# DoeringChristian/mitsuba3-experiments

Hardware: AMD Instinct MI355X
Metric: Mpaths/sec on bedroom@1280×720 spp=256, 1/2/4/8 GPUs; HBM GB/s vs peak (higher is better)
Workload: dtype f32; 1 GPU; path-mis.py NEE+MIS (BASELINE configs[1]) on bedroom-proxy 1280x720, global spp=256 split over 1 rank(s) by sample range, max_depth=8, rr_depth=2; global_spp=256, spp_per_rank=256, parallelism=sample-range shards x1

## Files before the change

mitsuba3-experiments_amd/csrc/context.cpp:

```cpp
#include <stdlib.h>
#include <string.h>

#include <algorithm>

#include "runtime.h"

namespace mtxh {

int dalloc(DevBuf &b, size_t bytes) {
  if (b.bytes >= bytes && b.p) return MTX_OK;
  if (b.p) hipFree(b.p);
  b.p = nullptr;
  b.bytes = 0;
  if (bytes == 0) return MTX_OK;
  hipError_t e = hipMalloc(&b.p, bytes);
  if (e != hipSuccess) {
    mtx_set_error("hipMalloc(%zu) failed: %s", bytes, hipGetErrorString(e));
    b.p = nullptr;
    return MTX_E_OOM;
  }
  b.bytes = bytes;
  return MTX_OK;
}

// ... 18 lines not shown
    if (p && !on_device(c, p)) {
      mtx_set_error("%s: argument %d is not device memory of device %d", fn, k, c->device);
      return MTX_E_ARG;
    }
    ++k;
  }
  return MTX_OK;
}

int stage(mtx_ctx *c, DevBuf &slot, size_t bytes, const void *src) {
  if (int rc = dalloc(slot, bytes)) return rc;
  if (src) HIP_TRY(hipMemcpyAsync(slot.p, src, bytes, hipMemcpyHostToDevice, c->stream));
  return MTX_OK;
}
int unstage(mtx_ctx *c, std::initializer_list<Unstage> outs) {
  for (const Unstage &o : outs) HIP_TRY(hipMemcpyAsync(o.dst, o.slot.p, o.bytes, hipMemcpyDeviceToHost, c->stream));
  HIP_TRY(hipStreamSynchronize(c->stream));
  return MTX_OK;
}

}

using namespace mtxh;

static bool read_knobs(Knobs &k) {
  if (const char *e = getenv("MTX_LDS_STACK")) k.lds_stack = std::max(1, std::min(MTX_BVH_MAX_DEPTH + 1, atoi(e)));
  if (const char *e = getenv("MTX_LDS_TOP")) k.lds_top = (uint32_t)std::max(0, std::min(256, atoi(e)));
  if (const char *e = getenv("MTX_OCC_LDS_TOP")) k.occ_lds_top = (uint32_t)std::max(0, std::min(192, atoi(e)));
  if (const char *e = getenv("MTX_OCC_LDS_STACK"))
    k.occ_lds_stack = std::max(1, std::min(MTX_BVH_MAX_DEPTH + 1, atoi(e)));
  if (const char *e = getenv("MTX_STREAMS_MAX_LOG2")) k.streams_max_log2 = (uint32_t)std::max(16, std::min(31, atoi(e)));
  if (const char *e = getenv("MTX_STREAMS")) k.streams = (uint32_t)std::max(1, std::min(2, atoi(e)));
  if (const char *e = getenv("MTX_TRACE_BATCH")) k.trace_batch = (uint32_t)std::max(1, std::min(1 << 16, atoi(e)));
  if (const char *e = getenv("MTX_UREFILL")) k.urefill = (uint32_t)std::max(1, std::min(64, atoi(e)));
  if (const char *e = getenv("MTX_CAM_UREFILL")) k.cam_urefill = (uint32_t)std::max(1, std::min(64, atoi(e)));
  if (const char *e = getenv("MTX_OCC_UREFILL")) k.occ_urefill = (uint32_t)std::max(1, std::min(64, atoi(e)));
  if (const char *e = getenv("MTX_TRACE_RING")) {
    char *end = nullptr;
    const long v = strtol(e, &end, 10);
    if (end == e || *end || !mtxd::ring_size_ok(v)) {
      mtx_set_error("MTX_TRACE_RING=%s: the ring holds 0 (none), 16 or 32 rays", e);
      return false;
    }
    k.trace_ring = (uint32_t)v;
  }
  if (const char *e = getenv("MTX_XCD_CLAIM")) k.xcd_claim = atoi(e) != 0;
  if (const char *e = getenv("MTX_RS_FUSED")) k.rs_fused = atoi(e) ? 1u : 0u;
  if (const char *e = getenv("MTX_MEGA_PATHS")) k.mega_paths = (uint32_t)strtoul(e, nullptr, 0);
  if (const char *e = getenv("MTX_CACHE_FUSED")) k.cache_fused = atoi(e) ? 1u : 0u;
  if (const char *e = getenv("MTX_ENCODE_LM")) k.encode_lm = atoi(e) ? 1u : 0u;
  if (const char *e = getenv("MTX_CACHE_SORT")) k.cache_sort = (uint32_t)std::max(0, std::min(2, atoi(e)));
  return true;
}

extern "C" {

int mtx_diag_shade_stamps(unsigned long long *out) { return mtxd::shade_stamps(out); }

int mtx_diag_trace_lds(uint32_t ring, uint32_t lds_stack, uint32_t lds_top, uint32_t *out) {
  if (!out || !mtxd::ring_size_ok(ring) || !lds_stack) return MTX_E_ARG;
  mtxd::DevScene s{};
  s.lds_entries = lds_stack;
  s.lds_top = lds_top;
  mtxd::split_trace_lds(s, ring);
  out[0] = (uint32_t)mtxd::ring_stack_bytes(s);
  out[1] = s.ring_lds_entries;
  return MTX_OK;
}

int mtx_ctx_create(int hip_device, mtx_ctx **out) {
  if (!out) {
    mtx_set_error("mtx_ctx_create: out is NULL");
    return MTX_E_ARG;
  }
  *out = nullptr;
  int n = 0;
  HIP_TRY(hipGetDeviceCount(&n));
  if (hip_device < 0 || hip_device >= n) {
    mtx_set_error("mtx_ctx_create: device %d out of range (%d devices)", hip_device, n);
    return MTX_E_ARG;
  }
  HIP_TRY(hipSetDevice(hip_device));
  hipDeviceProp_t prop;
  HIP_TRY(hipGetDeviceProperties(&prop, hip_device));
  if (strncmp(prop.gcnArchName, "gfx950", 6) != 0) {
    mtx_set_error("mtx_ctx_create: device %d is %s, libmtx is built for gfx950", hip_device, prop.gcnArchName);
    return MTX_E_UNSUPPORTED;
  }
  mtx_ctx *c = new mtx_ctx();
  c->device = hip_device;
  c->n_cu = prop.multiProcessorCount;
  hipError_t e = hipStreamCreateWithFlags(&c->stream, hipStreamNonBlocking);
  if (e != hipSuccess) {
    delete c;
    mtx_set_error("hipStreamCreate failed: %s", hipGetErrorString(e));
    return MTX_E_HIP;
  }
  c->wave[0].stream = c->stream;
  c->trace_grid = c->closest_grid = c->n_cu * 8;
  c->shade_grid = c->n_cu * mtxd::shade_blocks_per_cu();
  {
    int v = 0;
    c->max_lds = 160 * 1024;
    if (hipDeviceGetAttribute(&v, hipDeviceAttributeMaxSharedMemoryPerBlock, hip_device) == hipSuccess &&
        (size_t)v > c->max_lds)
      c->max_lds = (size_t)v;
  }
  if (!read_knobs(c->knobs)) {
    mtx_ctx_destroy(c);
    return MTX_E_ARG;
  }
  *out = c;
  return MTX_OK;
}

void mtx_ctx_destroy(mtx_ctx *c) {
  if (!c) return;
  hipSetDevice(c->device);
  for (Wave &w : c->wave)
    if (w.stream) hipStreamSynchronize(w.stream);
  Wave &w1 = c->wave[1];
  if (w1.start) hipEventDestroy(w1.start);
  if (w1.done) hipEventDestroy(w1.done);
  if (w1.stream) hipStreamDestroy(w1.stream);
  for (hipEvent_t ev : c->events) hipEventDestroy(ev);
  if (c->q_pinned) hipHostFree(c->q_pinned);
  for (hipEvent_t ev : c->prim_ev)
    if (ev) hipEventDestroy(ev);
  if (c->stream) hipStreamDestroy(c->stream);
  delete c;
}

double mtx_last_device_ms(mtx_ctx *c) { return c ? c->last_device_ms : 0.0; }

// ... 2 lines not shown
```

mitsuba3-experiments_amd/csrc/render.cpp:

```cpp
#include <string.h>

#include <algorithm>
#include <initializer_list>
#include <vector>

#include "runtime.h"
#include "mtx_core/film.h"
#include "prims.h"

namespace mtxh {

constexpr uint32_t kDefaultChunk = 1u << 28;
constexpr size_t kPathStateBytes = 328;
constexpr size_t kCacheQueryBytes = 3 * kQueryBytes + kFeatBytes + kOutBytes;
uint32_t default_chunk(mtx_ctx *c, const mtx_render_args *a, uint32_t ways, bool cache) {
  size_t free_b = 0, total_b = 0;
  if (hipMemGetInfo(&free_b, &total_b) != hipSuccess) return 1u << 22;
  const size_t per_path =
      kPathStateBytes + (cache ? kCacheQueryBytes : 0) +
      (a->integrator == MTX_INT_PSSMLT_SIMPLE ? 32ull * std::max<uint32_t>(a->max_depth, 1) + 48
       : a->integrator == MTX_INT_PSSMLT_PATH ? 48ull * std::max<uint32_t>(a->max_depth, 1) + 48
                                              : 0);
  const size_t held =
      ways > 1 ? std::min<size_t>(c->wave[0].capacity, c->wave[1].capacity) : c->wave[0].capacity;
// ... 191 lines not shown
      if (hipMemcpyAsync(&nq, b.cq_count, 4, hipMemcpyDeviceToHost, st) == hipSuccess &&
          hipStreamSynchronize(st) == hipSuccess)
        tm.cache_queries += nq;
    }
  }
  return MTX_OK;
}

void launch_bounce(mtx_ctx *c, const mtxd::WaveBuffers &b, const mtxd::ChunkParams &p, Timer &tm,
                   uint64_t *n_trace, uint64_t *n_shadow, const mtxd::DevScene &s, hipStream_t st, uint32_t bounce) {
  const bool nerad = p.integrator == MTX_INT_NERAD_RHS, nerad_render = p.integrator == MTX_INT_NERAD;
  hipEvent_t e;
  const int div = (nerad && bounce >= 2) ? 8 : 1;
  if (!(nerad && bounce == 0)) {
    e = tm.begin(0, st);
    if (bounce == 0 && p.cam0)
      mtxd::launch_trace_camera(s, b, p, std::max(1, c->closest_grid / div), st);
    else
      mtxd::launch_trace_closest(s, b, bounce, p.stats, std::max(1, c->closest_grid / div), st);
    tm.end(0, e, st);
    ++*n_trace;
  }
  e = tm.begin(2, st);
  mtxd::launch_shade(s, b, p, bounce, std::max(1, c->shade_grid / div), st);
  tm.end(2, e, st);
  if (p.integrator != MTX_INT_PSSMLT_SIMPLE && p.integrator != MTX_INT_SIMPLE && !nerad_render &&
      !(nerad && bounce > 0)) {
    e = tm.begin(1, st);
    mtxd::launch_trace_shadow(s, b, bounce, p.stats, c->trace_grid, st);
    tm.end(1, e, st);
    ++*n_shadow;
  }
}

uint32_t bounce_iters(const mtxd::ChunkParams &p) {
  return std::max<uint32_t>(p.max_depth, 1) + (p.nrc_cache ? 1u : 0u);
}

void finish_bounces(const mtxd::WaveBuffers &b, const mtxd::ChunkParams &p, hipStream_t st) {
  if (p.integrator != MTX_INT_NERAD_RHS && p.integrator != MTX_INT_NERAD)
    mtxd::launch_flush_tail(b, bounce_iters(p), b.capacity, p.integrator, st);
}

void run_bounces(mtx_ctx *c, const Wave &w, const mtxd::WaveBuffers &b, const mtxd::ChunkParams &p, Timer &tm,
                 uint64_t *n_trace, uint64_t *n_shadow) {
  const mtxd::DevScene s = wave_scene(c, w);
  hipStream_t st = w.stream;
// ... 665 lines not shown
```

mitsuba3-experiments_amd/csrc/runtime.h:

```cpp
#pragma once
#include <hip/hip_runtime.h>
#include <stdint.h>

#include <initializer_list>
#include <utility>
#include <vector>

#include "mtx.h"
#include "mtx_core/field.h"
#include "mtx_core/nerad.h"
#include "refit.h"
#include "wavefront.h"

void mtx_set_error(const char *fmt, ...);

#define HIP_TRY(expr)                                                                             \
  do {                                                                                            \
    hipError_t e_ = (expr);                                                                       \
    if (e_ != hipSuccess) {                                                                       \
      mtx_set_error("%s failed: %s (%s:%d)", #expr, hipGetErrorString(e_), __FILE__, __LINE__); \
      return MTX_E_HIP;                                                                           \
    }                                                                                             \
  } while (0)

// ... 46 lines not shown
struct Wave {
  hipStream_t stream = nullptr;
  hipEvent_t start = nullptr, done = nullptr;
  DevBuf plane[kNumPlanes];
  DevBuf counters, xheads;
  DevBuf stack_ovf;
  DevBuf cq_p, cq_d, cq_t, cq_count, f_feat, f_out;
  DevBuf cq_perm, cq_cursor;
  uint32_t capacity = 0;
};

struct Knobs {
  uint32_t streams = MTX_STREAMS;
  uint32_t streams_max_log2 = 27;
  uint32_t lds_stack = mtxd::kLdsStack;
  uint32_t lds_top = MTX_LDS_TOP;
  uint32_t occ_lds_top = MTX_OCC_LDS_TOP;
  uint32_t occ_lds_stack = mtxd::kOccLdsStack;
  uint32_t trace_batch = 128;
  uint32_t urefill = 24;
  uint32_t cam_urefill = 64;
  uint32_t occ_urefill = 12;
  uint32_t trace_ring = MTX_TRACE_RING;
  uint32_t xcd_claim = 1;
  uint32_t mega_paths = 0xffffffffu;
  uint32_t rs_fused = 1;
  uint32_t cache_sort = MTX_CACHE_SORT;
  uint32_t encode_lm = MTX_ENCODE_LM;
  uint32_t cache_fused = 1;
};

struct SceneState {
  DevBuf shade_rec;
  DevBuf nodes, tri, occ_nodes, occ_tri, tri_vidx, tri_shape, vpos, vnormal, vuv, shapes, materials, emitters, textures,
      texels, tables;
  mtxd::DevScene dev{};
  uint32_t n_shapes = 0;
  uint32_t n_materials = 0;
  uint32_t n_nodes = 0, n_occ = 0, n_verts = 0, n_tables = 0;
  bool live = false;
};

struct RefitState {
  DevBuf occ_perm, lvl4_list, lvl8_list;
  std::vector<uint32_t> lvl4_first, lvl8_first;
  DevBuf state, tbox, nbox, vpos, vnormal;
// ... 160 lines not shown
```

mitsuba3-experiments_amd/csrc/scene.cpp:

```cpp
#include <string.h>

#include <algorithm>
#include <vector>

#include "runtime.h"
#include "mtx_core/interaction.h"
#include "scene_check.h"

using namespace mtxh;

static int upload_levels(const std::vector<uint32_t> &level, uint32_t depth, std::vector<uint32_t> &first,
                         DevBuf &list, hipStream_t st) {
  first.assign((size_t)depth + 1, 0u);
  bool contiguous = true;
  uint32_t prev = 0;
  for (uint32_t l : level) {
    if (l >= depth) {
      contiguous = false;
      continue;
    }
    ++first[l + 1];
    contiguous = contiguous && l >= prev;
    prev = l;
  }
  for (uint32_t l = 0; l < depth; ++l) first[l + 1] += first[l];
  if (contiguous) {
    dfree(list);
    return MTX_OK;
  }
// ... 89 lines not shown
    t.pmf = (float *)c->refit.em_pmf.p;
    t.cdf = (float *)c->refit.em_cdf.p;
    t.bsum = (double *)c->refit.em_bsum.p;
    t.bstat = (uint32_t *)c->refit.em_bstat.p;
  }
  {
    std::vector<float> rec(32 * (size_t)d->n_tris, 0.f);
    for (uint32_t t = 0; t < d->n_tris; ++t) {
      float *r = &rec[32 * (size_t)t];
      const mtx_shape &sh = d->shapes[d->tri_shape[t]];
      const uint32_t use_n = (!(sh.flags & 1u) && d->vnormal) ? 1u : 0u;
      const uint32_t use_uv = ((sh.flags & 2u) && d->vuv) ? 2u : 0u;
      for (int k = 0; k < 3; ++k) {
        const uint32_t vi = d->tri_vidx[3 * (size_t)t + k];
        for (int a = 0; a < 3; ++a) r[4 * k + a] = d->vpos[3 * (size_t)vi + a];
        if (use_n)
          for (int a = 0; a < 3; ++a) r[12 + 4 * k + a] = d->vnormal[3 * (size_t)vi + a];
        if (use_uv) {
          r[24 + 2 * k] = d->vuv[2 * (size_t)vi];
          r[24 + 2 * k + 1] = d->vuv[2 * (size_t)vi + 1];
        }
      }
      const mtx_material &m = d->materials[sh.material];
      const uint32_t cls = 1u + ((m.type & 7u) << 2 | (m.tex >= 0 ? 2u : 0u) | ((m.flags & MTX_MF_MASK) ? 1u : 0u));
      const uint32_t mat = sh.material, fl = use_n | use_uv | (cls << 8);
      const int32_t em = sh.emitter;
      memcpy(&r[3], &mat, 4);
      memcpy(&r[7], &em, 4);
      memcpy(&r[11], &fl, 4);
    }
    if ((rc = upload(c->scene.shade_rec, rec.data(), rec.size(), st))) return rc;
    HIP_TRY(hipStreamSynchronize(st));
  }
  HIP_TRY(hipStreamSynchronize(st));
  mtxd::DevScene &s = c->scene.dev;
  s.nodes = (const int4 *)c->scene.nodes.p;
  s.tri = (const float *)c->scene.tri.p;
  s.occ_nodes = (const int4 *)c->scene.occ_nodes.p;
  s.occ_tri = (const float *)c->scene.occ_tri.p;
  s.tri_vidx = (const uint32_t *)c->scene.tri_vidx.p;
  s.tri_shape = (const uint32_t *)c->scene.tri_shape.p;
  s.vpos = (const float *)c->scene.vpos.p;
  s.vnormal = (const float *)c->scene.vnormal.p;
  s.vuv = (const float *)c->scene.vuv.p;
  s.shapes = (const mtx_shape *)c->scene.shapes.p;
  s.shade_rec = (const float4 *)c->scene.shade_rec.p;
  s.materials = (const mtx_material *)c->scene.materials.p;
// ... 133 lines not shown
  if (e == hipSuccess) e = hipStreamSynchronize(st);
  if (e == hipSuccess) e = hipGetLastError();
  if (e != hipSuccess || (flags & mtxd::RF_BAD_QUANT)) {
    c->scene_dropped();
    if (e != hipSuccess) {
      mtx_set_error("mtx_scene_update_vertices: %s; the scene was dropped, upload it again", hipGetErrorString(e));
      return MTX_E_HIP;
    }
    mtx_set_error("mtx_scene_update_vertices: child box quantisation failed; the scene was dropped, upload it again");
    return MTX_E_ARG;
  }
  mtx::V3 lo, hi;
  lo.x = mtxd::refit_key_decode(h[mtxd::RF_LO]);
  lo.y = mtxd::refit_key_decode(h[mtxd::RF_LO + 1]);
  lo.z = mtxd::refit_key_decode(h[mtxd::RF_LO + 2]);
  hi.x = mtxd::refit_key_decode(h[mtxd::RF_HI]);
  hi.y = mtxd::refit_key_decode(h[mtxd::RF_HI + 1]);
  hi.z = mtxd::refit_key_decode(h[mtxd::RF_HI + 2]);
  mtx::env_bsphere_box(lo, hi, c->scene.dev.env_center, &c->scene.dev.env_radius);
  c->geometry_moved();
  return MTX_OK;
}

int mtx_scene_read(mtx_ctx *c, int which, void *out, uint64_t n_bytes) {
  if (!c || !out) {
    mtx_set_error("mtx_scene_read: null argument");
    return MTX_E_ARG;
  }
  if (!c->scene.live) {
    mtx_set_error("no scene uploaded");
    return MTX_E_NOSCENE;
  }
  const uint64_t nt = c->scene.dev.n_tris, nv = c->scene.n_verts;
  const void *src = nullptr;
  uint64_t need = 0;
  switch (which) {
    case 0: src = c->scene.nodes.p; need = 4ull * MTX_BVH_NODE_WORDS * c->scene.n_nodes; break;
    case 1: src = c->scene.occ_nodes.p; need = 4ull * MTX_OCC_NODE_WORDS * c->scene.n_occ; break;
    case 2: src = c->scene.tri.p; need = 36 * nt; break;
    case 3: src = c->scene.occ_tri.p; need = 36 * nt; break;
    case 4: src = c->scene.shade_rec.p; need = 128 * nt; break;
    case 5: src = c->scene.vpos.p; need = 12 * nv; break;
    case 6: src = c->scene.vnormal.p; need = c->scene.vnormal.p ? 12 * nv : 0; break;
    case 7: need = 16; break;
    case 8: src = c->scene.tables.p; need = 4ull * c->scene.n_tables; break;
    case 9: src = c->scene.emitters.p; need = sizeof(mtx_emitter) * (uint64_t)c->scene.dev.n_emitters; break;
// ... 22 lines not shown
```

mitsuba3-experiments_amd/csrc/shade.hip:

```cpp
#include <hip/hip_runtime.h>

#include <algorithm>

#include "device_common.h"
#include "shade_dev.h"

#ifndef MTX_SHADE_MIN_BLOCKS
#define MTX_SHADE_MIN_BLOCKS 3
#endif
constexpr int kShadeMinBlocks = MTX_SHADE_MIN_BLOCKS;

namespace mtxd {

__global__ void k_raygen_camera(DevScene s, WaveBuffers b, ChunkParams p) {
  const uint32_t i = blockIdx.x * blockDim.x + threadIdx.x;
  if (i == 0) b.counters[0] = p.n_paths;
  if (i >= p.n_paths) return;
  const CamPath cp = camera_path(s.camera, s.has_env != 0, p, i);
  init_path(b, p, i, cp.ray, cp.rng, cp.pos, s.has_env != 0);
}

__global__ void k_raygen_rays(DevScene s, WaveBuffers b, ChunkParams p, const float *rays, const uint32_t *lanes,
                              uint32_t rng_skip) {
  const uint32_t i = blockIdx.x * blockDim.x + threadIdx.x;
  if (i == 0) b.counters[0] = p.n_paths;
  if (i >= p.n_paths) return;
  Pcg32 rng = sampler_lane(p.seed, lanes[i]);
  for (uint32_t k = 0; k < rng_skip; ++k) rng.next_u32();
  const float *r = rays + 6 * (size_t)i;
  Ray ray{V3{r[0], r[1], r[2]}, V3{r[3], r[4], r[5]}, kLargest};
  init_path(b, p, i, ray, rng, make_float2(0.f, 0.f), s.has_env != 0);
}

#if MTX_DIAG_STAMPS
__device__ unsigned long long g_shade_stamps[kStampSegs + 2];
#endif

template <int INT, bool CAM>
__device__ __forceinline__ void shade_loop(const DevScene &s, const WaveBuffers &b, const ChunkParams &p,
                                           uint32_t bounce_) {
  const uint32_t bounce = CAM ? 0u : bounce_;
  const SceneView sv = make_view(s);
  const uint32_t count = b.counters[4 * bounce + 0];
  const uint32_t *in_q = b.queue[bounce & 1];
  uint32_t *out_q = b.queue[(bounce + 1) & 1];
  uint32_t *out_cnt = &b.counters[4 * (bounce + 1) + 0];
  const uint32_t rp = (bounce + b.ray_par) & 1u;
  constexpr bool kNerad = INT == MTX_INT_NERAD_RHS || INT == MTX_INT_NERAD;
  const uint32_t stride = gridDim.x * kShadeBlock;
  uint32_t parity = 0;
  uint32_t path = 0;
  float4 h = make_float4(0.f, 0.f, 0.f, 0.f);
  const bool ident = bounce == 0 && p.ident0;
  if (blockIdx.x * kShadeBlock + threadIdx.x < count) {
    const uint32_t i0 = blockIdx.x * kShadeBlock + threadIdx.x;
    path = ident ? i0 : ld_stream<kNtQueue>(in_q + i0);
    h = ld_stream<kNtShade>(b.hit + i0);
  }

  Stamps stp{};
  MTX_STAMP_BEGIN(stp);
  for (uint32_t base = blockIdx.x * kShadeBlock; base < count; base += stride, parity ^= 1u) {
    const uint32_t i = base + threadIdx.x;
    const uint32_t inext = i + stride;
    uint32_t path_n = 0;
    if (inext < count) path_n = ident ? inext : ld_stream<kNtQueue>(in_q + inext);
    float4 hn = make_float4(0.f, 0.f, 0.f, 0.f);
    if (inext < count) hn = b.hit[inext];
    const uint32_t pn = __float_as_uint(hn.y);
    const float4 *wp = (inext < count && pn != 0xffffffffu) ? s.shade_rec + 8 * (size_t)pn : nullptr;
    ShadeIO io;
    io.reset();
    MTX_STAMP_STEP(stp);
    io.st = stp;
    bool cont = false;
    const bool valid = i < count;
    if (valid) {
      if constexpr (INT == MTX_INT_PSSMLT_SIMPLE)
        cont = shade_pssmlt(s, sv, b, p, bounce, path, i, h, io);
      else if constexpr (INT == MTX_INT_SIMPLE)
        cont = shade_simple<CAM>(s, sv, b, p, bounce, path, i, h, io);
      else if constexpr (INT == MTX_INT_PSSMLT_PATH)
        cont = shade_pssmlt_path(s, sv, b, p, bounce, path, i, h, io);
      else if constexpr (INT == MTX_INT_NERAD_RHS)
        cont = shade_nerad<false>(s, sv, b, bounce, path, i, h, io);
      else if constexpr (INT == MTX_INT_NERAD)
        cont = shade_nerad<true>(s, sv, b, bounce, path, i, h, io);
      else
        cont = shade_path<INT, CAM>(s, sv, b, p, bounce, path, i, h, io, wp);
    }
    (void)wp;
    const uint32_t path_c = path;
    path = path_n;
    h = hn;
    asm volatile("" ::"v"(io.warm));
    stp = io.st;

    uint32_t slot, sslot;
    block_append2<kShadeBlock>(cont, io.emit, io.emit && io.em_hi, out_cnt, parity, slot, sslot);
    MTX_STAMP(stp, 6);
    if (cont) {
      st_stream<kNtQueue>(out_q + slot, path_c);
      st_stream<kNtShadeSt>(b.ray_o[rp ^ 1u] + slot, io.nro);
      st_stream<kNtShadeSt>(b.ray_d[rp ^ 1u] + slot, io.nrd);
      if constexpr (!kNerad) st_stream<kNtShadeSt>(b.thr[rp ^ 1u] + slot, io.nthr);
      if constexpr (INT == MTX_INT_PATH_MIS || INT == MTX_INT_PATH || INT == MTX_INT_NRC || INT == MTX_INT_PSSMLT_PATH)
        st_stream<kNtShadeSt>(b.prev[rp ^ 1u] + slot, io.nprev);
      if constexpr (!kNerad) {
        st_stream<kNtShadeSt>(b.L[rp ^ 1u] + slot, io.nL);
        st_stream<kNtShadeSt>(b.misc[rp ^ 1u] + slot, io.nmisc);
      }
    } else if (!kNerad && valid) {
      st_stream<kNtShadeSt>(b.L[kFinal] + path_c, io.nL);
      if (!p.drop_end_misc) st_stream<kNtShadeSt>(b.misc[kFinal] + path_c, io.nmisc);
    }
    if (io.emit) {
      const uint32_t li = (kNerad || !cont) ? kFinal * b.capacity + path_c : (rp ^ 1u) * b.capacity + slot;
      io.rec.d.w = __uint_as_float(li);
// ... 7 lines not shown
    if constexpr (INT == MTX_INT_NRC || INT == MTX_INT_NERAD_RHS || INT == MTX_INT_NERAD) {
      if (INT != MTX_INT_NRC || p.nrc_cache) {
        const uint32_t q = block_reserve<kShadeBlock>(io.query ? 1u : 0u, b.cq_count);
        if (io.query) {
          b.cq_p[q] = io.qp;
          b.cq_d[q] = io.qd;
          b.cq_t[q] = io.qt;
        }
      }
    }
    MTX_STAMP(stp, 8);
  }
#if MTX_DIAG_STAMPS
  if ((threadIdx.x & 63u) == 0) {
    for (int k = 0; k < kStampSegs; ++k) atomicAdd(&g_shade_stamps[k], stp.acc[k]);
    atomicAdd(&g_shade_stamps[kStampSegs], stp.steps);
    atomicAdd(&g_shade_stamps[kStampSegs + 1], 1ull);
  }
#endif
}

template <int INT>
__global__ __launch_bounds__(kShadeBlock, kShadeMinBlocks) void k_shade(DevScene s, WaveBuffers b, ChunkParams p, uint32_t bounce) {
  shade_loop<INT, false>(s, b, p, bounce);
}
template <int INT>
__global__ __launch_bounds__(kShadeBlock, kShadeMinBlocks) void k_shade_cam(DevScene s, WaveBuffers b, ChunkParams p) {
  static_assert(INT == MTX_INT_PATH || INT == MTX_INT_PATH_MIS || INT == MTX_INT_NRC || INT == MTX_INT_SIMPLE,
                "k_shade_cam: the integrators whose bounce-0 shade derives the camera sample");
  shade_loop<INT, true>(s, b, p, 0u);
}

__global__ void k_flush_tail(WaveBuffers b, uint32_t bounce, uint32_t integrator) {
  const uint32_t n = b.counters[4 * bounce];
  const uint32_t *q = b.queue[bounce & 1];
  const uint32_t rp = (bounce + b.ray_par) & 1u;
  for (uint32_t k = blockIdx.x * blockDim.x + threadIdx.x; k < n; k += gridDim.x * blockDim.x) {
    const uint32_t path = q[k];
    float4 L = b.L[rp][k];
    const uint4 m = b.misc[rp][k];
    if (integrator == MTX_INT_PATH_MIS || integrator == MTX_INT_RESTIR_GI) L.w = end_w(m.w >> 16);
    b.L[kFinal][path] = L;
    b.misc[kFinal][path] = m;
  }
}

// ... 83 lines not shown
    cur.y = po.y;
    b.mlt_L[i] = f4(Lp, 0.f);
    for (uint32_t d = 0; d < dirty; ++d)
      b.vpath[(size_t)d * b.capacity + i] = b.vprop[(size_t)d * b.capacity + i];
    if (p.integrator == MTX_INT_PSSMLT_PATH)
      for (uint32_t d = 0; d < dirty; ++d)
        b.vpath_es[(size_t)d * b.capacity + i] = b.vprop_es[(size_t)d * b.capacity + i];
    dirty = 0;
  }
  cur.w = (float)dirty;
  b.mlt_cur[i] = cur;
  b.misc[kFinal][i] = st_rng(rng, 0u);
}

void launch_raygen_camera(const DevScene &s, const WaveBuffers &b, const ChunkParams &p, hipStream_t st) {
  hipLaunchKernelGGL(k_raygen_camera, dim3(blocks_for(p.n_paths, 256)), dim3(256), 0, st, s, b, p);
}
void launch_raygen_rays(const DevScene &s, const WaveBuffers &b, const ChunkParams &p, const float *rays,
                        const uint32_t *lanes, uint32_t rng_skip, hipStream_t st) {
  hipLaunchKernelGGL(k_raygen_rays, dim3(blocks_for(p.n_paths, 256)), dim3(256), 0, st, s, b, p, rays, lanes,
                     rng_skip);
}
void launch_shade(const DevScene &s, const WaveBuffers &b, const ChunkParams &p, uint32_t bounce, int grid,
                  hipStream_t st) {
  if (bounce == 0 && p.cam0) {
    switch (p.integrator) {
      case MTX_INT_PATH:
        hipLaunchKernelGGL(k_shade_cam<MTX_INT_PATH>, dim3(grid), dim3(kShadeBlock), 0, st, s, b, p);
        break;
      case MTX_INT_NRC:
        hipLaunchKernelGGL(k_shade_cam<MTX_INT_NRC>, dim3(grid), dim3(kShadeBlock), 0, st, s, b, p);
        break;
      case MTX_INT_SIMPLE:
        hipLaunchKernelGGL(k_shade_cam<MTX_INT_SIMPLE>, dim3(grid), dim3(kShadeBlock), 0, st, s, b, p);
        break;
      default:
        hipLaunchKernelGGL(k_shade_cam<MTX_INT_PATH_MIS>, dim3(grid), dim3(kShadeBlock), 0, st, s, b, p);
    }
    return;
  }
  switch (p.integrator) {
    case MTX_INT_PATH:
      hipLaunchKernelGGL(k_shade<MTX_INT_PATH>, dim3(grid), dim3(kShadeBlock), 0, st, s, b, p, bounce);
      break;
    case MTX_INT_NRC:
      hipLaunchKernelGGL(k_shade<MTX_INT_NRC>, dim3(grid), dim3(kShadeBlock), 0, st, s, b, p, bounce);
      break;
    case MTX_INT_PSSMLT_SIMPLE:
      hipLaunchKernelGGL(k_shade<MTX_INT_PSSMLT_SIMPLE>, dim3(grid), dim3(kShadeBlock), 0, st, s, b, p, bounce);
      break;
    case MTX_INT_SIMPLE:
      hipLaunchKernelGGL(k_shade<MTX_INT_SIMPLE>, dim3(grid), dim3(kShadeBlock), 0, st, s, b, p, bounce);
      break;
    case MTX_INT_PSSMLT_PATH:
      hipLaunchKernelGGL(k_shade<MTX_INT_PSSMLT_PATH>, dim3(grid), dim3(kShadeBlock), 0, st, s, b, p, bounce);
      break;
    case MTX_INT_NERAD_RHS:
      hipLaunchKernelGGL(k_shade<MTX_INT_NERAD_RHS>, dim3(grid), dim3(kShadeBlock), 0, st, s, b, p, bounce);
      break;
    case MTX_INT_NERAD:
      hipLaunchKernelGGL(k_shade<MTX_INT_NERAD>, dim3(grid), dim3(kShadeBlock), 0, st, s, b, p, bounce);
      break;
    default:
      hipLaunchKernelGGL(k_shade<MTX_INT_PATH_MIS>, dim3(grid), dim3(kShadeBlock), 0, st, s, b, p, bounce);
  }
}
int shade_stamps(unsigned long long *out) {
#if MTX_DIAG_STAMPS
  if (hipDeviceSynchronize() != hipSuccess) return -1;
  if (hipMemcpyFromSymbol(out, HIP_SYMBOL(g_shade_stamps), sizeof(unsigned long long) * (kStampSegs + 2)) !=
      hipSuccess)
    return -1;
  unsigned long long z[kStampSegs + 2] = {};
  if (hipMemcpyToSymbol(HIP_SYMBOL(g_shade_stamps), z, sizeof(z)) != hipSuccess) return -1;
  return kStampSegs;
#else
  (void)out;
  return -1;
#endif
}
int shade_blocks_per_cu() {
  int nb = 0;
  if (hipOccupancyMaxActiveBlocksPerMultiprocessor(&nb, k_shade<MTX_INT_PATH_MIS>, kShadeBlock, 0) != hipSuccess ||
      nb <= 0)
    nb = 2;
  return nb;
}
void launch_cache_apply(const WaveBuffers &b, const float *out, uint32_t capacity, hipStream_t st,
                        const uint32_t *perm) {
  const unsigned blocks = (unsigned)std::min<uint64_t>((capacity + 255) / 256, 16384);
  hipLaunchKernelGGL(k_cache_apply, dim3(std::max(1u, blocks)), dim3(256), 0, st, b, out, perm);
}
void launch_flush_tail(const WaveBuffers &b, uint32_t bounce, uint32_t capacity, uint32_t integrator,
                       hipStream_t st) {
  const unsigned blocks = (unsigned)std::min<uint64_t>((capacity + 255) / 256, 1024);
  hipLaunchKernelGGL(k_flush_tail, dim3(std::max(1u, blocks)), dim3(256), 0, st, b, bounce, integrator);
}
void launch_mlt_init(const WaveBuffers &b, const ChunkParams &p, hipStream_t st) {
  hipLaunchKernelGGL(k_mlt_init, dim3(blocks_for(p.n_paths, 256)), dim3(256), 0, st, b, p, p.max_depth);
}
void launch_mlt_begin(const DevScene &s, const WaveBuffers &b, const ChunkParams &p, hipStream_t st) {
  hipLaunchKernelGGL(k_mlt_begin, dim3(blocks_for(p.n_paths, 256)), dim3(256), 0, st, s, b, p);
}
void launch_mlt_end(const WaveBuffers &b, const ChunkParams &p, hipStream_t st) {
  hipLaunchKernelGGL(k_mlt_end, dim3(blocks_for(p.n_paths, 256)), dim3(256), 0, st, b, p, p.max_depth);
}

// ... 10 lines not shown
```

mitsuba3-experiments_amd/csrc/wavefront.h:

```cpp
#pragma once
#include <hip/hip_runtime.h>
#include <stdint.h>

#include "mtx.h"
#include "mtx_core/nerad.h"

namespace mtxd {

enum : uint32_t {
  PF_VALID_RAY = 1u,
  PF_PREV_DELTA = 2u,
  PF_PRIMARY_VALID = 4u,
  PF_CACHE_QUERY = 8u,
};

#ifndef MTX_TRACE_BLOCK
#define MTX_TRACE_BLOCK 256
#endif
constexpr int kTraceBlock = MTX_TRACE_BLOCK;
constexpr int kShadeBlock = 256;
constexpr uint32_t kLdsStack = 16;
constexpr uint32_t kOccLdsStack = 8;
#ifndef MTX_LDS_TOP
#define MTX_LDS_TOP 64
#endif
#ifndef MTX_OCC_LDS_TOP
#define MTX_OCC_LDS_TOP 48
#endif
#ifndef MTX_TRACE_RING
#define MTX_TRACE_RING 32
#endif
constexpr bool ring_size_ok(long R) { return R == 0 || R == 16 || R == 32; }
static_assert(ring_size_ok(MTX_TRACE_RING), "MTX_TRACE_RING: 0, 16 or 32");
constexpr uint32_t kTraceLds = 20 * 1024;
constexpr uint32_t kRingWords = 14;
constexpr uint32_t ring_bytes(uint32_t R) { return R * 4u * kRingWords * (kTraceBlock / 64u); }
#ifndef MTX_CACHE_SORT
#define MTX_CACHE_SORT 2
#endif
#ifndef MTX_ENCODE_LM
#define MTX_ENCODE_LM 1
#endif
#ifndef MTX_CAM0
#define MTX_CAM0 1
#endif
#ifndef MTX_STREAMS
#define MTX_STREAMS 2
#endif

constexpr uint32_t kXcds = 8;
constexpr uint32_t kXHeadStride = 32;
constexpr uint32_t kXSlotWords = kXcds * kXHeadStride;

struct DevScene {
  const int4 *nodes;
  const float *tri;
  const int4 *occ_nodes;
  const float *occ_tri;
  const uint32_t *tri_vidx;
// ... 116 lines not shown
struct ChunkParams {
  uint32_t integrator, max_depth, rr_depth, seed;
  uint32_t spp, spp_total, sample_offset;
  uint32_t width, height;
  uint32_t px0, n_px;
  uint32_t band_y0;
  uint32_t band_px;
  uint32_t rfilter;
  uint32_t film_slots;
  uint32_t slot_mask;
  uint32_t n_paths;
  float nrc_c;
  uint32_t stats;
  uint32_t large_step;
  uint32_t restir;
  uint32_t nrc_cache;
  uint32_t drop_end_misc;
  uint32_t ident0;
  uint32_t cam0;
};

int trace_blocks_per_cu(const DevScene &s);
int closest_blocks_per_cu(const DevScene &s);
int shade_blocks_per_cu();
int mega_blocks_per_cu(const DevScene &s);
void launch_path_mega(const DevScene &s, const WaveBuffers &b, const ChunkParams &p, int grid, hipStream_t st);
void launch_rs_stage_a(const DevScene &s, const WaveBuffers &b, const ChunkParams &p, const RestirBuffers &r,
                       int grid, hipStream_t st);
int shade_stamps(unsigned long long *out);
void launch_raygen_camera(const DevScene &s, const WaveBuffers &b, const ChunkParams &p, hipStream_t st);
void launch_raygen_rays(const DevScene &s, const WaveBuffers &b, const ChunkParams &p, const float *rays,
                        const uint32_t *lanes, uint32_t rng_skip, hipStream_t st);
void launch_trace_closest(const DevScene &s, const WaveBuffers &b, uint32_t bounce, uint32_t stats, int grid,
                          hipStream_t st);
void launch_trace_camera(const DevScene &s, const WaveBuffers &b, const ChunkParams &p, int grid, hipStream_t st);
void launch_trace_shadow(const DevScene &s, const WaveBuffers &b, uint32_t bounce, uint32_t stats, int grid,
                         hipStream_t st);
void launch_shade(const DevScene &s, const WaveBuffers &b, const ChunkParams &p, uint32_t bounce, int grid,
                  hipStream_t st);
void launch_film_src(const WaveBuffers &b, const ChunkParams &p, float4 *contrib, hipStream_t st);
void launch_film_gather(const float4 *contrib, float4 *film, uint32_t width, uint32_t y0, uint32_t y1,
                        uint32_t nslots, uint32_t slot_mask, uint32_t rfilter, hipStream_t st);
void launch_mlt_init(const WaveBuffers &b, const ChunkParams &p, hipStream_t st);
void launch_mlt_begin(const DevScene &s, const WaveBuffers &b, const ChunkParams &p, hipStream_t st);
void launch_mlt_end(const WaveBuffers &b, const ChunkParams &p, hipStream_t st);
void launch_mlt_film(const WaveBuffers &b, const ChunkParams &p, float4 *contrib, hipStream_t st);
void launch_flush_tail(const WaveBuffers &b, uint32_t bounce, uint32_t capacity, uint32_t integrator,
                       hipStream_t st);
void launch_collect(const WaveBuffers &b, const ChunkParams &p, float *L_out, uint8_t *valid_out, hipStream_t st);
void launch_cache_apply(const WaveBuffers &b, const float *out, uint32_t capacity, hipStream_t st,
                        const uint32_t *perm = nullptr);
void launch_restir_begin(const DevScene &s, const WaveBuffers &b, const ChunkParams &p, const RestirBuffers &r,
                         hipStream_t st);
void launch_restir_collect(const WaveBuffers &b, const ChunkParams &p, const RestirBuffers &r, hipStream_t st);
void launch_restir_temporal(const RestirBuffers &r, const ChunkParams &p, hipStream_t st);
void launch_restir_spatial_rays(const RestirBuffers &r, const ChunkParams &p, hipStream_t st);
void launch_restir_spatial_merge(const RestirBuffers &r, const ChunkParams &p, hipStream_t st);
void launch_restir_bias_finish(const RestirBuffers &r, const ChunkParams &p, hipStream_t st);
void launch_restir_final(const DevScene &s, const WaveBuffers &b, const ChunkParams &p, const RestirBuffers &r,
                         hipStream_t st);
void launch_trace_test(const DevScene &s, const RestirBuffers &r, uint32_t occ_base, int grid, hipStream_t st);
void launch_trace_raw(const DevScene &s, const float4 *rays, uint32_t n, int any_hit, uint32_t *hits,
// ... 10 lines not shown
```

Before: 1546 Mpaths/s.

## Bin shade work into per-material-class LDS ring queues to cut divergence

Adds an in-block compaction scheme to the shade kernel for path and path-mis integrators. Each block ballots incoming hits by material class (diffuse, roughplastic, other), stages them in per-class LDS rings, and shades a full block of a single class whenever one fills, flushing mixed leftovers at the end. The aim is to cut wavefront divergence across material BSDF code paths. In exchange it adds LDS use that can lower occupancy, extra block barriers per batch, and it drops the next-item prefetch of the mixed loop. It is on by default and can be disabled with an env knob.

After: 1760 Mpaths/s, median of 6. 13.9% higher.

```diff
diff --git a/include/mtx_core/shade_class.h b/include/mtx_core/shade_class.h
--- /dev/null
+++ b/include/mtx_core/shade_class.h
@@ -0,0 +1,21 @@
+#pragma once
+#include "../mtx.h"
+#include "common.h"
+
+namespace mtx {
+
+constexpr uint32_t kShadeClasses = 3;
+
+MTX_HD uint32_t shade_class_of_type(uint32_t type) {
+  return type == MTX_MAT_DIFFUSE ? 0u : type == MTX_MAT_ROUGHPLASTIC ? 1u : 2u;
+}
+
+MTX_HD uint32_t shade_rec_class_bits(uint32_t type, bool textured, bool masked) {
+  return 1u + ((type & 7u) << 2 | (textured ? 2u : 0u) | (masked ? 1u : 0u));
+}
+MTX_HD uint32_t shade_class_of_rec(uint32_t flag_word) {
+  const uint32_t c = (flag_word >> 8) & 0x1fu;
+  return c ? shade_class_of_type((c - 1u) >> 2) : 0u;
+}
+
+}
diff --git a/mitsuba3-experiments_amd/csrc/context.cpp b/mitsuba3-experiments_amd/csrc/context.cpp
--- a/mitsuba3-experiments_amd/csrc/context.cpp
+++ b/mitsuba3-experiments_amd/csrc/context.cpp
@@ -64,6 +64,15 @@
 }
 
 using namespace mtxh;
+
+static bool shade_classes_knob(const char *e, uint32_t *out) {
+  if (!e || !(e[0] == '0' || e[0] == '1') || e[1]) {
+    mtx_set_error("MTX_SHADE_CLASSES=%s: 0 (the mixed shade loop) or 1 (class queues)", e ? e : "(null)");
+    return false;
+  }
+  *out = (uint32_t)(e[0] - '0');
+  return true;
+}
 
 static bool read_knobs(Knobs &k) {
   if (const char *e = getenv("MTX_LDS_STACK")) k.lds_stack = std::max(1, std::min(MTX_BVH_MAX_DEPTH + 1, atoi(e)));
@@ -86,6 +95,9 @@
     }
     k.trace_ring = (uint32_t)v;
   }
+  if (const char *e = getenv("MTX_SHADE_CLASSES")) {
+    if (!shade_classes_knob(e, &k.shade_classes)) return false;
+  }
   if (const char *e = getenv("MTX_XCD_CLAIM")) k.xcd_claim = atoi(e) != 0;
   if (const char *e = getenv("MTX_RS_FUSED")) k.rs_fused = atoi(e) ? 1u : 0u;
   if (const char *e = getenv("MTX_MEGA_PATHS")) k.mega_paths = (uint32_t)strtoul(e, nullptr, 0);
@@ -98,6 +110,8 @@
 extern "C" {
 
 int mtx_diag_shade_stamps(unsigned long long *out) { return mtxd::shade_stamps(out); }
+
+int mtx_diag_shade_class_mix(unsigned long long *out) { return mtxd::shade_class_mix(out); }
 
 int mtx_diag_trace_lds(uint32_t ring, uint32_t lds_stack, uint32_t lds_top, uint32_t *out) {
   if (!out || !mtxd::ring_size_ok(ring) || !lds_stack) return MTX_E_ARG;
@@ -110,6 +124,22 @@
   return MTX_OK;
 }
 
+uint32_t mtx_diag_shade_class_of_type(uint32_t type) { return mtx::shade_class_of_type(type); }
+int mtx_diag_shade_classes_knob(const char *value, uint32_t *out) {
+  if (!out || !shade_classes_knob(value, &out[0])) return MTX_E_ARG;
+  out[1] = mtxd::shade_class_lds_bytes();
+  out[2] = mtxd::kClassRing;
+  out[3] = mtx::kShadeClasses;
+  return MTX_OK;
+}
+
+int mtx_diag_shade_grid(const mtx_ctx *c, uint32_t *out) {
+  if (!c || !out) return MTX_E_ARG;
+  out[0] = (uint32_t)c->shade_grid;
+  out[1] = (uint32_t)c->n_cu;
+  return MTX_OK;
+}
+
 int mtx_ctx_create(int hip_device, mtx_ctx **out) {
   if (!out) {
     mtx_set_error("mtx_ctx_create: out is NULL");
@@ -140,7 +170,6 @@
   }
   c->wave[0].stream = c->stream;
   c->trace_grid = c->closest_grid = c->n_cu * 8;
-  c->shade_grid = c->n_cu * mtxd::shade_blocks_per_cu();
   {
     int v = 0;
     c->max_lds = 160 * 1024;
@@ -152,6 +181,7 @@
     mtx_ctx_destroy(c);
     return MTX_E_ARG;
   }
+  c->shade_grid = c->n_cu * mtxd::shade_blocks_per_cu(c->knobs.shade_classes != 0);
   *out = c;
   return MTX_OK;
 }
diff --git a/mitsuba3-experiments_amd/csrc/render.cpp b/mitsuba3-experiments_amd/csrc/render.cpp
--- a/mitsuba3-experiments_amd/csrc/render.cpp
+++ b/mitsuba3-experiments_amd/csrc/render.cpp
@@ -237,7 +237,7 @@
     ++*n_trace;
   }
   e = tm.begin(2, st);
-  mtxd::launch_shade(s, b, p, bounce, std::max(1, c->shade_grid / div), st);
+  mtxd::launch_shade(s, b, p, bounce, std::max(1, c->shade_grid / div), st, c->knobs.shade_classes != 0);
   tm.end(2, e, st);
   if (p.integrator != MTX_INT_PSSMLT_SIMPLE && p.integrator != MTX_INT_SIMPLE && !nerad_render &&
       !(nerad && bounce > 0)) {
diff --git a/mitsuba3-experiments_amd/csrc/runtime.h b/mitsuba3-experiments_amd/csrc/runtime.h
--- a/mitsuba3-experiments_amd/csrc/runtime.h
+++ b/mitsuba3-experiments_amd/csrc/runtime.h
@@ -92,6 +92,7 @@
   uint32_t cam_urefill = 64;
   uint32_t occ_urefill = 12;
   uint32_t trace_ring = MTX_TRACE_RING;
+  uint32_t shade_classes = MTX_SHADE_CLASSES;
   uint32_t xcd_claim = 1;
   uint32_t mega_paths = 0xffffffffu;
   uint32_t rs_fused = 1;
diff --git a/mitsuba3-experiments_amd/csrc/scene.cpp b/mitsuba3-experiments_amd/csrc/scene.cpp
--- a/mitsuba3-experiments_amd/csrc/scene.cpp
+++ b/mitsuba3-experiments_amd/csrc/scene.cpp
@@ -5,6 +5,7 @@
 
 #include "runtime.h"
 #include "mtx_core/interaction.h"
+#include "mtx_core/shade_class.h"
 #include "scene_check.h"
 
 using namespace mtxh;
@@ -140,7 +141,7 @@
         }
       }
       const mtx_material &m = d->materials[sh.material];
-      const uint32_t cls = 1u + ((m.type & 7u) << 2 | (m.tex >= 0 ? 2u : 0u) | ((m.flags & MTX_MF_MASK) ? 1u : 0u));
+      const uint32_t cls = mtx::shade_rec_class_bits(m.type, m.tex >= 0, (m.flags & MTX_MF_MASK) != 0);
       const uint32_t mat = sh.material, fl = use_n | use_uv | (cls << 8);
       const int32_t em = sh.emitter;
       memcpy(&r[3], &mat, 4);
@@ -320,6 +321,24 @@
   return MTX_OK;
 }
 
+int mtx_diag_shade_classes(const mtx_scene_desc *d, uint8_t *out) {
+  if (!d || !out || !d->tri_shape || !d->shapes || !d->materials) {
+    mtx_set_error("mtx_diag_shade_classes: null argument");
+    return MTX_E_ARG;
+  }
+  for (uint32_t t = 0; t < d->n_tris; ++t) {
+    const uint32_t sh = d->tri_shape[t];
+    if (sh >= d->n_shapes || d->shapes[sh].material >= d->n_materials) {
+      mtx_set_error("mtx_diag_shade_classes: triangle %u: shape or material out of range", t);
+      return MTX_E_ARG;
+    }
+    const mtx_material &m = d->materials[d->shapes[sh].material];
+    const uint32_t fl = mtx::shade_rec_class_bits(m.type, m.tex >= 0, (m.flags & MTX_MF_MASK) != 0) << 8;
+    out[t] = (uint8_t)mtx::shade_class_of_rec(fl);
+  }
+  return MTX_OK;
+}
+
 int mtx_scene_read(mtx_ctx *c, int which, void *out, uint64_t n_bytes) {
   if (!c || !out) {
     mtx_set_error("mtx_scene_read: null argument");
diff --git a/mitsuba3-experiments_amd/csrc/shade.hip b/mitsuba3-experiments_amd/csrc/shade.hip
--- a/mitsuba3-experiments_amd/csrc/shade.hip
+++ b/mitsuba3-experiments_amd/csrc/shade.hip
@@ -36,9 +36,34 @@
 __device__ unsigned long long g_shade_stamps[kStampSegs + 2];
 #endif
 
-template <int INT, bool CAM>
+#ifndef MTX_DIAG_CLASSES
+#define MTX_DIAG_CLASSES 0
+#endif
+#if MTX_DIAG_CLASSES
+constexpr uint32_t kMixBounces = 16, kMixWords = 2 * mtx::kShadeClasses;
+__device__ unsigned long long g_class_mix[kMixBounces][kMixWords];
+__device__ __forceinline__ void class_mix_count(const DevScene &s, uint32_t bounce, bool valid, const float4 h) {
+  const uint32_t prim = __float_as_uint(h.y);
+  uint32_t cw = 0;
+  if (valid && prim != 0xffffffffu) cw = __float_as_uint(s.shade_rec[8 * (size_t)prim + 2].w);
+  const uint32_t cls = mtx::shade_class_of_rec(cw);
+  uint32_t held = 0, n[mtx::kShadeClasses];
+  for (uint32_t k = 0; k < mtx::kShadeClasses; ++k) {
+    n[k] = (uint32_t)__popcll(__ballot(valid && cls == k));
+    held += n[k] ? 1u : 0u;
+  }
+  if ((threadIdx.x & 63u) == 0 && held && bounce < kMixBounces) {
+    atomicAdd(&g_class_mix[bounce][held - 1], 1ull);
+    for (uint32_t k = 0; k < mtx::kShadeClasses; ++k)
+      atomicAdd(&g_class_mix[bounce][mtx::kShadeClasses + k], (unsigned long long)n[k]);
+  }
+}
+#endif
+
+template <int INT, bool CAM, bool CLS = false>
 __device__ __forceinline__ void shade_loop(const DevScene &s, const WaveBuffers &b, const ChunkParams &p,
                                            uint32_t bounce_) {
+  static_assert(!CLS || (shade_has_classes(INT) && !CAM), "class queues: k_shade of path-mis and path");
   const uint32_t bounce = CAM ? 0u : bounce_;
   const SceneView sv = make_view(s);
   const uint32_t count = b.counters[4 * bounce + 0];
@@ -57,43 +82,163 @@
     path = ident ? i0 : ld_stream<kNtQueue>(in_q + i0);
     h = ld_stream<kNtShade>(b.hit + i0);
   }
+  constexpr uint32_t kC = mtx::kShadeClasses, kW = kShadeBlock / 64, kMask = kClassRing - 1;
+  static_assert((kClassRing & kMask) == 0 && kClassRing >= 2 * kShadeBlock, "a ring holds two block steps");
+  static_assert(kClassEntryBytes == sizeof(float4) + sizeof(uint2), "ring entry: hit record | position, path");
+  extern __shared__ float4 class_lds[];
+  float4 *ring_h = class_lds;
+  uint2 *ring_ip = reinterpret_cast<uint2 *>(class_lds + kC * kClassRing);
+  __shared__ uint32_t class_wcnt[CLS ? kW : 1][kC];
+  uint32_t head[kC] = {}, fill[kC] = {};
+  uint32_t nbase = blockIdx.x * kShadeBlock, cw = 0;
+  bool cw_due = CLS && nbase < count;
+  auto load_class_word = [&]() {
+    const uint32_t pn = __float_as_uint(h.y);
+    cw = 0;
+    if (nbase + threadIdx.x < count && pn != 0xffffffffu) cw = __float_as_uint(s.shade_rec[8 * (size_t)pn + 2].w);
+    cw_due = false;
+  };
 
   Stamps stp{};
   MTX_STAMP_BEGIN(stp);
-  for (uint32_t base = blockIdx.x * kShadeBlock; base < count; base += stride, parity ^= 1u) {
-    const uint32_t i = base + threadIdx.x;
-    const uint32_t inext = i + stride;
-    uint32_t path_n = 0;
-    if (inext < count) path_n = ident ? inext : ld_stream<kNtQueue>(in_q + inext);
-    float4 hn = make_float4(0.f, 0.f, 0.f, 0.f);
-    if (inext < count) hn = b.hit[inext];
-    const uint32_t pn = __float_as_uint(hn.y);
-    const float4 *wp = (inext < count && pn != 0xffffffffu) ? s.shade_rec + 8 * (size_t)pn : nullptr;
+  for (uint32_t base = blockIdx.x * kShadeBlock; CLS || base < count; base += CLS ? 0u : stride, parity ^= 1u) {
+    uint32_t i = base + threadIdx.x, path_s = path, path_n = 0;
+    float4 h_s = h, hn = make_float4(0.f, 0.f, 0.f, 0.f);
+    bool valid = i < count;
+    const float4 *wp = nullptr;
+    if constexpr (!CLS) {
+      const uint32_t inext = i + stride;
+      if (inext < count) path_n = ident ? inext : ld_stream<kNtQueue>(in_q + inext);
+      if (inext < count) hn = b.hit[inext];
+      const uint32_t pn = __float_as_uint(hn.y);
+      wp = (inext < count && pn != 0xffffffffu) ? s.shade_rec + 8 * (size_t)pn : nullptr;
+    } else {
+      const uint32_t wave = threadIdx.x >> 6;
+      uint32_t c, most, held;
+      for (;;) {
+        c = 0;
+        most = held = fill[0];
+#pragma unroll
+        for (uint32_t k = 1; k < kC; ++k) {
+          if (fill[k] > most) {
+            most = fill[k];
+            c = k;
+          }
+          held += fill[k];
+        }
+        if (most >= (uint32_t)kShadeBlock || nbase >= count) break;
+        if (cw_due) load_class_word();
+        const uint32_t i_n = nbase + threadIdx.x;
+        const bool in = i_n < count;
+        const uint32_t cls = mtx::shade_class_of_rec(cw);
+        uint64_t m[kC];
+#pragma unroll
+        for (uint32_t k = 0; k < kC; ++k) m[k] = __ballot(in && cls == k);
+        if ((threadIdx.x & 63u) == 0) {
+#pragma unroll
+          for (uint32_t k = 0; k < kC; ++k) class_wcnt[wave][k] = (uint32_t)__popcll(m[k]);
+        }
+        __syncthreads();
+        uint32_t slot = 0;
+#pragma unroll
+        for (uint32_t k = 0; k < kC; ++k) {
+          uint32_t before = 0, total = 0;
+#pragma unroll
+          for (uint32_t w = 0; w < kW; ++w) {
+            const uint32_t n = __builtin_amdgcn_readfirstlane(class_wcnt[w][k]);
+            if (w < wave) before += n;
+            total += n;
+          }
+          const uint32_t rank = before + __builtin_amdgcn_mbcnt_hi((uint32_t)(m[k] >> 32),
+                                                                   __builtin_amdgcn_mbcnt_lo((uint32_t)m[k], 0u));
+          if (cls == k) slot = k * kClassRing + ((head[k] + fill[k] + rank) & kMask);
+          fill[k] += total;
+        }
+        if (in) {
+          ring_h[slot] = h;
+          ring_ip[slot] = make_uint2(i_n, path);
+        }
+        nbase += stride;
+        if (nbase + threadIdx.x < count) {
+          path = ident ? nbase + threadIdx.x : ld_stream<kNtQueue>(in_q + nbase + threadIdx.x);
+          h = b.hit[nbase + threadIdx.x];
+        }
+        cw_due = nbase < count;
+        __syncthreads();
+      }
+      if (held == 0) break;
+      valid = false;
+      if (most >= (uint32_t)kShadeBlock) {
+        uint32_t hc = 0;
+#pragma unroll
+        for (uint32_t k = 0; k < kC; ++k)
+          if (c == k) {
+            hc = head[k];
+            head[k] = (head[k] + kShadeBlock) & kMask;
+            fill[k] -= kShadeBlock;
+          }
+        const uint32_t slot = c * kClassRing + ((hc + threadIdx.x) & kMask);
+        const uint2 ip = ring_ip[slot];
+        h_s = ring_h[slot];
+        i = ip.x;
+        path_s = ip.y;
+        valid = true;
+      } else {
+        uint32_t t = threadIdx.x, room = kShadeBlock;
+#pragma unroll
+        for (uint32_t k = 0; k < kC; ++k) {
+          const uint32_t take = fill[k] < room ? fill[k] : room;
+          if (!valid && t < take) {
+            const uint32_t slot = k * kClassRing + ((head[k] + t) & kMask);
+            const uint2 ip = ring_ip[slot];
+            h_s = ring_h[slot];
+            i = ip.x;
+            path_s = ip.y;
+            valid = true;
+          }
+          t -= take;
+          head[k] = (head[k] + take) & kMask;
+          fill[k] -= take;
+          room -= take;
+        }
+      }
+#pragma unroll
+      for (uint32_t k = 0; k < kC; ++k) {
+        head[k] = __builtin_amdgcn_readfirstlane(head[k]);
+        fill[k] = __builtin_amdgcn_readfirstlane(fill[k]);
+      }
+    }
     ShadeIO io;
     io.reset();
     MTX_STAMP_STEP(stp);
     io.st = stp;
     bool cont = false;
-    const bool valid = i < count;
+#if MTX_DIAG_CLASSES
+    if constexpr (!CAM && !CLS && shade_has_classes(INT)) class_mix_count(s, bounce, valid, h_s);
+#endif
     if (valid) {
       if constexpr (INT == MTX_INT_PSSMLT_SIMPLE)
-        cont = shade_pssmlt(s, sv, b, p, bounce, path, i, h, io);
+        cont = shade_pssmlt(s, sv, b, p, bounce, path_s, i, h_s, io);
       else if constexpr (INT == MTX_INT_SIMPLE)
-        cont = shade_simple<CAM>(s, sv, b, p, bounce, path, i, h, io);
+        cont = shade_simple<CAM>(s, sv, b, p, bounce, path_s, i, h_s, io);
       else if constexpr (INT == MTX_INT_PSSMLT_PATH)
-        cont = shade_pssmlt_path(s, sv, b, p, bounce, path, i, h, io);
+        cont = shade_pssmlt_path(s, sv, b, p, bounce, path_s, i, h_s, io);
       else if constexpr (INT == MTX_INT_NERAD_RHS)
-        cont = shade_nerad<false>(s, sv, b, bounce, path, i, h, io);
+        cont = shade_nerad<false>(s, sv, b, bounce, path_s, i, h_s, io);
       else if constexpr (INT == MTX_INT_NERAD)
-        cont = shade_nerad<true>(s, sv, b, bounce, path, i, h, io);
+        cont = shade_nerad<true>(s, sv, b, bounce, path_s, i, h_s, io);
       else
-        cont = shade_path<INT, CAM>(s, sv, b, p, bounce, path, i, h, io, wp);
+        cont = shade_path<INT, CAM>(s, sv, b, p, bounce, path_s, i, h_s, io, wp);
     }
     (void)wp;
-    const uint32_t path_c = path;
-    path = path_n;
-    h = hn;
-    asm volatile("" ::"v"(io.warm));
+    const uint32_t path_c = path_s;
+    if constexpr (!CLS) {
+      path = path_n;
+      h = hn;
+      asm volatile("" ::"v"(io.warm));
+    } else {
+      if (cw_due) load_class_word();
+    }
     stp = io.st;
 
     uint32_t slot, sslot;
@@ -147,6 +292,11 @@
 
 template <int INT>
 __global__ __launch_bounds__(kShadeBlock, kShadeMinBlocks) void k_shade(DevScene s, WaveBuffers b, ChunkParams p, uint32_t bounce) {
+  shade_loop<INT, false, shade_has_classes(INT)>(s, b, p, bounce);
+}
+template <int INT>
+__global__ __launch_bounds__(kShadeBlock, kShadeMinBlocks) void k_shade_mixed(DevScene s, WaveBuffers b, ChunkParams p, uint32_t bounce) {
+  static_assert(shade_has_classes(INT), "k_shade_mixed: the integrators whose k_shade runs class queues");
   shade_loop<INT, false>(s, b, p, bounce);
 }
 template <int INT>
@@ -276,7 +426,8 @@
                      rng_skip);
 }
 void launch_shade(const DevScene &s, const WaveBuffers &b, const ChunkParams &p, uint32_t bounce, int grid,
-                  hipStream_t st) {
+                  hipStream_t st, bool classes) {
+  const size_t rings = shade_class_lds_bytes();
   if (bounce == 0 && p.cam0) {
     switch (p.integrator) {
       case MTX_INT_PATH:
@@ -295,7 +446,10 @@
   }
   switch (p.integrator) {
     case MTX_INT_PATH:
-      hipLaunchKernelGGL(k_shade<MTX_INT_PATH>, dim3(grid), dim3(kShadeBlock), 0, st, s, b, p, bounce);
+      if (classes)
+        hipLaunchKernelGGL(k_shade<MTX_INT_PATH>, dim3(grid), dim3(kShadeBlock), rings, st, s, b, p, bounce);
+      else
+        hipLaunchKernelGGL(k_shade_mixed<MTX_INT_PATH>, dim3(grid), dim3(kShadeBlock), 0, st, s, b, p, bounce);
       break;
     case MTX_INT_NRC:
       hipLaunchKernelGGL(k_shade<MTX_INT_NRC>, dim3(grid), dim3(kShadeBlock), 0, st, s, b, p, bounce);
@@ -316,7 +470,10 @@
       hipLaunchKernelGGL(k_shade<MTX_INT_NERAD>, dim3(grid), dim3(kShadeBlock), 0, st, s, b, p, bounce);
       break;
     default:
-      hipLaunchKernelGGL(k_shade<MTX_INT_PATH_MIS>, dim3(grid), dim3(kShadeBlock), 0, st, s, b, p, bounce);
+      if (classes)
+        hipLaunchKernelGGL(k_shade<MTX_INT_PATH_MIS>, dim3(grid), dim3(kShadeBlock), rings, st, s, b, p, bounce);
+      else
+        hipLaunchKernelGGL(k_shade_mixed<MTX_INT_PATH_MIS>, dim3(grid), dim3(kShadeBlock), 0, st, s, b, p, bounce);
   }
 }
 int shade_stamps(unsigned long long *out) {
@@ -333,10 +490,27 @@
   return -1;
 #endif
 }
-int shade_blocks_per_cu() {
+int shade_class_mix(unsigned long long *out) {
+#if MTX_DIAG_CLASSES
+  if (hipDeviceSynchronize() != hipSuccess) return -1;
+  if (hipMemcpyFromSymbol(out, HIP_SYMBOL(g_class_mix), sizeof(unsigned long long) * kMixBounces * kMixWords) !=
+      hipSuccess)
+    return -1;
+  unsigned long long z[kMixBounces * kMixWords] = {};
+  if (hipMemcpyToSymbol(HIP_SYMBOL(g_class_mix), z, sizeof(z)) != hipSuccess) return -1;
+  return (int)kMixWords;
+#else
+  (void)out;
+  return -1;
+#endif
+}
+int shade_blocks_per_cu(bool classes) {
   int nb = 0;
-  if (hipOccupancyMaxActiveBlocksPerMultiprocessor(&nb, k_shade<MTX_INT_PATH_MIS>, kShadeBlock, 0) != hipSuccess ||
-      nb <= 0)
+  const hipError_t e =
+      classes ? hipOccupancyMaxActiveBlocksPerMultiprocessor(&nb, k_shade<MTX_INT_PATH_MIS>, kShadeBlock,
+                                                             shade_class_lds_bytes())
+              : hipOccupancyMaxActiveBlocksPerMultiprocessor(&nb, k_shade_mixed<MTX_INT_PATH_MIS>, kShadeBlock, 0);
+  if (e != hipSuccess || nb <= 0)
     nb = 2;
   return nb;
 }
diff --git a/mitsuba3-experiments_amd/csrc/wavefront.h b/mitsuba3-experiments_amd/csrc/wavefront.h
--- a/mitsuba3-experiments_amd/csrc/wavefront.h
+++ b/mitsuba3-experiments_amd/csrc/wavefront.h
@@ -4,6 +4,7 @@
 
 #include "mtx.h"
 #include "mtx_core/nerad.h"
+#include "mtx_core/shade_class.h"
 
 namespace mtxd {
 
@@ -35,6 +36,15 @@
 constexpr uint32_t kTraceLds = 20 * 1024;
 constexpr uint32_t kRingWords = 14;
 constexpr uint32_t ring_bytes(uint32_t R) { return R * 4u * kRingWords * (kTraceBlock / 64u); }
+#ifndef MTX_SHADE_CLASSES
+#define MTX_SHADE_CLASSES 1
+#endif
+constexpr uint32_t kClassRing = 2 * kShadeBlock;
+constexpr uint32_t kClassEntryBytes = 24;
+constexpr uint32_t shade_class_lds_bytes() { return mtx::kShadeClasses * kClassRing * kClassEntryBytes; }
+constexpr bool shade_has_classes(int integrator) {
+  return integrator == MTX_INT_PATH_MIS || integrator == MTX_INT_PATH;
+}
 #ifndef MTX_CACHE_SORT
 #define MTX_CACHE_SORT 2
 #endif
@@ -197,12 +207,13 @@
 
 int trace_blocks_per_cu(const DevScene &s);
 int closest_blocks_per_cu(const DevScene &s);
-int shade_blocks_per_cu();
+int shade_blocks_per_cu(bool classes);
 int mega_blocks_per_cu(const DevScene &s);
 void launch_path_mega(const DevScene &s, const WaveBuffers &b, const ChunkParams &p, int grid, hipStream_t st);
 void launch_rs_stage_a(const DevScene &s, const WaveBuffers &b, const ChunkParams &p, const RestirBuffers &r,
                        int grid, hipStream_t st);
 int shade_stamps(unsigned long long *out);
+int shade_class_mix(unsigned long long *out);
 void launch_raygen_camera(const DevScene &s, const WaveBuffers &b, const ChunkParams &p, hipStream_t st);
 void launch_raygen_rays(const DevScene &s, const WaveBuffers &b, const ChunkParams &p, const float *rays,
                         const uint32_t *lanes, uint32_t rng_skip, hipStream_t st);
@@ -212,7 +223,7 @@
 void launch_trace_shadow(const DevScene &s, const WaveBuffers &b, uint32_t bounce, uint32_t stats, int grid,
                          hipStream_t st);
 void launch_shade(const DevScene &s, const WaveBuffers &b, const ChunkParams &p, uint32_t bounce, int grid,
-                  hipStream_t st);
+                  hipStream_t st, bool classes);
 void launch_film_src(const WaveBuffers &b, const ChunkParams &p, float4 *contrib, hipStream_t st);
 void launch_film_gather(const float4 *contrib, float4 *film, uint32_t width, uint32_t y0, uint32_t y1,
                         uint32_t nslots, uint32_t slot_mask, uint32_t rfilter, hipStream_t st);
```
